# HaoxiangYou/Q_Learning_with_HJB

Measured on AMD Instinct MI355X. Metric: env-steps/sec (batched HJB rollouts), cartpole batch=2^20, higher is better.
Workload: dtype f32; 1 GPU; cartpole balancing + vhjb controller (BASELINE configs[1]); batch_per_gpu=1048576, global_batch=1048576, state_dim=4, control_dim=1, integrator=euler, mlp=4-128-128-64 relu, no bias, parallelism=env-shard x1, no data-path collective

## Files before the change

q_learning_with_hjb_amd/csrc/hjbx_mlp.hip:

```cpp
#include <hip/hip_runtime.h>
#include <type_traits>

#include <cstddef>

#include "hjbx_internal.hpp"
#include "hjbx_systems.hpp"
#include "hjbx_host.hpp"
#include "hjbx_mlp_core.hpp"
#include "hjbx_mlp_x3.hpp"
#include "hjbx_mlp_h2.hpp"
#include "hjbx_mlp_kernels.hpp"
#include "hjbx_mlp_host.hpp"

using namespace hjbx;

#ifndef HJBX_MLP_ACT
#error "compile hjbx_mlp.hip with -DHJBX_MLP_ACT=0 (relu + the C entry points), =1 (tanh), =2 (relu, bf16x3-split MFMA), =3 (relu, f16x2-split MFMA) and =4 (sin)"
#endif
static constexpr int kArith = HJBX_MLP_ACT == 2 ? 1 : HJBX_MLP_ACT == 3 ? 2 : 0;
static constexpr int kAct = kArith ? HJBX_ACT_RELU : HJBX_MLP_ACT == 4 ? HJBX_ACT_SIN : HJBX_MLP_ACT;
static_assert(kAct == HJBX_ACT_RELU || kAct == HJBX_ACT_TANH || kAct == HJBX_ACT_SIN, "fused kernels exist for relu, tanh and sin");
#define HJBX_MLP_CAT2(a, b) a##b
#define HJBX_MLP_CAT(a, b) HJBX_MLP_CAT2(a, b)
#define HJBX_MLP_SYM(name) HJBX_MLP_CAT(name, HJBX_MLP_ACT)
// ... 102 lines not shown
        return hjbx_user_value_grad(sys, &net, x, V, g, B, stream, "hjbx_value_grad_f32");
    }
    if (mlp->activation == HJBX_ACT_TANH) return hjbx_mlp_value_grad_act1(sys, mlp, x, V, g, B, stream);
    if (mlp->activation == HJBX_ACT_SIN) return hjbx_mlp_value_grad_act4(sys, mlp, x, V, g, B, stream);
    const int arith = hjbx_option_value(HJBX_OPT_MLP_ARITHMETIC);
    return arith == 1 ? hjbx_mlp_value_grad_act2(sys, mlp, x, V, g, B, stream)
         : arith == 2 ? hjbx_mlp_value_grad_act3(sys, mlp, x, V, g, B, stream)
                      : hjbx_mlp_value_grad_act0(sys, mlp, x, V, g, B, stream);
}
#endif

template <typename S>
static int launch_vhjb_rollout(const hjbx_system* sysh, S sys, const hjbx_task* task, const hjbx_mlp* mlp, int integrator, int t_first,
                               int n_steps, int T_max, const float* x, float* traj, float* u_log, float* cost, float* done, float* resid,
                               int32_t* done_step, float* x_out, const int32_t* order, int64_t B, void* workspace, void* st) {
    constexpr int N = S::N, M = S::M;
    constexpr int WAVES = HJBX_MLP_WAVES;
    const MlpP<N> p = make_mlp_params<N>(mlp->mean, mlp->std, mlp->xf, mlp->eps_scalar);
    const auto tk = make_task<float, N, M>(task);
    const auto lim = make_limits<float, M>(sysh);
    RolloutOut<N, M> o{traj, u_log, cost, done, resid, done_step, x_out};
    int64_t ngroups = 0, grid = 0;
    int sched = 0;
    if (int rc = mlp_rollout_grid(B, &ngroups, &grid, &sched, "hjbx_vhjb_rollout_f32")) return rc;
    const float *W1 = (const float*)mlp->W1, *W2 = (const float*)mlp->W2, *W3 = (const float*)mlp->W3;
    auto launch = [&](auto integ) {
        hipLaunchKernelGGL((k_vhjb_rollout_mfma<decltype(integ)::value, S, WAVES, kAct, kArith>), dim3((unsigned)grid), dim3(WAVES * 64), 0,
                           (hipStream_t)st, sys, p, tk, lim, W1, W2, W3, t_first, n_steps, T_max, x, order, o, B, ngroups, (unsigned*)workspace, sched, MlpHeadPd{});
    };
    if (integrator == HJBX_EULER) launch(std::integral_constant<int, 0>{});
    else if (integrator == HJBX_RK4) launch(std::integral_constant<int, 1>{});
    else if constexpr (S::kHasZoh) launch(std::integral_constant<int, 2>{});
    hipError_t e = hipGetLastError();
    if (e != hipSuccess) return hjbx_set_error(HJBX_EHIP, "hjbx_vhjb_rollout_f32: %s", hipGetErrorString(e));
    return HJBX_OK;
}

int HJBX_MLP_SYM(hjbx_mlp_rollout_act)(const hjbx_system* sys, const hjbx_task* task, const hjbx_mlp* mlp, int integrator, int t_first, int n_steps,
                                       int T_max, const float* x, float* traj, float* u_log, float* cost, float* done, float* resid,
                                       int32_t* done_step, float* x_out, const int32_t* env_order, int64_t B, void* workspace, void* stream) {
    int rc = HJBX_EUNSUPPORTED;
#ifdef HJBX_MLP_DEV
    if (sys->kind == HJBX_SYS_CARTPOLE && integrator == HJBX_EULER) {
        Cartpole<float> S{(float)sys->p[0], (float)sys->p[1], (float)sys->p[2], (float)sys->p[3]};
        constexpr int WAVES = HJBX_MLP_WAVES;
        MlpP<4> p;
        for (int k = 0; k < 4; ++k) { p.mean[k] = (float)mlp->mean[k]; p.istd[k] = (float)(1.0 / mlp->std[k]); p.xf[k] = (float)mlp->xf[k]; }
        p.eps_s = (float)mlp->eps_scalar;
        RolloutOut<4, 1> o{traj, u_log, cost, done, resid, done_step, x_out};
        const int64_t ngroups = (B + 31) / 32;
        int64_t grid = ngroups < 256 ? ngroups : 256;
        hipLaunchKernelGGL((k_vhjb_rollout_mfma<0, Cartpole<float>, WAVES, kAct, kArith>), dim3((unsigned)grid), dim3(WAVES * 64), 0, (hipStream_t)stream, S, p,
                           make_task<float, 4, 1>(task), make_limits<float, 1>(sys), (const float*)mlp->W1, (const float*)mlp->W2, (const float*)mlp->W3, t_first,
                           n_steps, T_max, x, env_order, o, B, ngroups, (unsigned*)workspace, hjbx_option_value(HJBX_OPT_ROLLOUT_SCHEDULE), MlpHeadPd{});
        return hipGetLastError() == hipSuccess ? HJBX_OK : hjbx_set_error(HJBX_EHIP, "launch");
    }
    return hjbx_set_error(HJBX_EUNSUPPORTED, "hjbx_vhjb_rollout_f32: development build (cartpole, Euler only)");
#else
    const bool ok = with_system<float>(sys, [&](auto S) {
        using SS = decltype(S);
        if constexpr (SS::N % 2 == 0)
            rc = launch_vhjb_rollout<SS>(sys, S, task, mlp, integrator, t_first, n_steps, T_max, x, traj, u_log, cost, done, resid, done_step,
                                         x_out, env_order, B, workspace, stream);
    });
    if (!ok || rc == HJBX_EUNSUPPORTED)
        return hjbx_set_error(HJBX_EUNSUPPORTED, "hjbx_vhjb_rollout_f32: no kernel for system kind %d with n=%d m=%d", sys->kind, sys->n, sys->m);
    return rc;
#endif
}

#if HJBX_MLP_ACT == 0
extern "C" int hjbx_vhjb_rollout_f32(const hjbx_system* sys, const hjbx_task* task, const hjbx_mlp* mlp, int integrator, int t_first,
                                     int n_steps, int T_max, const float* x, float* traj, float* u_log, float* cost, float* done,
// ... 40 lines not shown
```

q_learning_with_hjb_amd/csrc/hjbx_mlp_core.hpp:

```cpp
#pragma once
#include <hip/hip_runtime.h>

#include <cstddef>

#include "hjbx_internal.hpp"
#include "hjbx_systems.hpp"

using namespace hjbx;

using f32x16 = __attribute__((ext_vector_type(16))) float;
using f32x2 = __attribute__((ext_vector_type(2))) float;

static constexpr int kH1 = 128, kH2 = 128, kH3 = 64;
static constexpr int kLD1 = 129, kLD2 = 129, kLD3 = 65;

template <int N> struct MlpP { float mean[N], istd[N], xf[N], eps_s; };

__device__ __forceinline__ constexpr int perm(int s) { return (s & 3) + 8 * (s >> 2); }

#define MFMA(a, b, c) __builtin_amdgcn_mfma_f32_32x32x2f32((a), (b), (c), 0, 0, 0)

__device__ __forceinline__ float relu1(float v) {
    const int b = __builtin_bit_cast(int, v);
    return __builtin_bit_cast(float, b > 0 ? b : 0);
// ... 161 lines not shown
__device__ __forceinline__ void mlp_fill_bias(MlpBias& L, const float* __restrict__ b1g, const float* __restrict__ b2g, const float* __restrict__ b3g,
                                              const float* __restrict__ w4g, const float* __restrict__ b4g, int tid) {
    for (int idx = tid; idx < kH1; idx += THREADS) L.b1[idx] = b1g[idx];
    for (int idx = tid; idx < kH2; idx += THREADS) L.b2[idx] = b2g[idx];
    for (int idx = tid; idx < kH3; idx += THREADS) { L.b3[idx] = b3g[idx]; L.w4[idx] = w4g[idx]; }
    if (tid == 0) L.b4 = b4g[0];
}

template <int N> __device__ __forceinline__ MlpCtx mlp_ctx(MlpLds<N>& L, int lane) {
    constexpr int NP = MlpLds<N>::NP;
    MlpCtx c;
    c.i = lane & 31;
    c.h = lane >> 5;
    const uint32_t lds0 = (uint32_t)(uintptr_t)&L;
    c.w1f = lds0 + (uint32_t)offsetof(MlpLds<N>, W1) + 4u * (c.h * kLD1 + c.i);
    c.w2f = lds0 + (uint32_t)offsetof(MlpLds<N>, W2) + 4u * (4 * c.h * kLD2 + c.i);
    c.w3f = lds0 + (uint32_t)offsetof(MlpLds<N>, W3) + 4u * (4 * c.h * kLD3 + c.i);
    c.w3b = lds0 + (uint32_t)offsetof(MlpLds<N>, W3) + 4u * (c.i * kLD3 + 4 * c.h);
    c.w2b = lds0 + (uint32_t)offsetof(MlpLds<N>, W2) + 4u * (c.i * kLD2 + 4 * c.h);
    c.w1t = reinterpret_cast<const float4*>(L.W1T + 4 * c.h * NP);
    return c;
}

template <typename S, int TL, int ACT = HJBX_ACT_RELU, bool SOFT = false>
__device__ __forceinline__ void mlp_value_grad(const S& sys, const MlpP<S::N>& p, const MlpCtx& c, const float (&xs)[TL][S::N],
                                               bool want_grad, float (&V)[TL], float (&g)[TL][S::N], const MlpBias* bias = nullptr) {
    constexpr int N = S::N;
    constexpr int NP = MlpLds<N>::NP;
    const int h = c.h;
    float e[TL][N], z[TL][N], ee[TL];
#pragma unroll
    for (int t = 0; t < TL; ++t) {
        ee[t] = 0.f;
#pragma unroll
        for (int k = 0; k < N; ++k) e[t][k] = xs[t][k] - p.xf[k];
        sys.wrap(e[t]);
#pragma unroll
        for (int k = 0; k < N; ++k) {
            ee[t] += e[t][k] * e[t][k];
            z[t][k] = (e[t][k] - p.mean[k]) * p.istd[k];
        }
    }
    float ring4[3][4], ring2[3][2];

    f32x16 a1[TL][4];
    if constexpr (SOFT) bias_acc(a1, bias->b1, h);
    else zero_acc(a1);
    mfma_chain<OffW1F, N / 2, 4, 2, TL>(a1, ring4, c.w1f, [&](int st, int t) { return h ? z[t][2 * st + 1] : z[t][2 * st]; });


#pragma unroll
    for (int t = 0; t < TL; ++t)
#pragma unroll
        for (int fb = 0; fb < 4; ++fb)
#pragma unroll
            for (int r = 0; r < 16; ++r) {
                a1[t][fb][r] = act1<ACT>(a1[t][fb][r]);
                if constexpr (ACT == HJBX_ACT_SIN) {
                    asm volatile("" : "+v"(a1[t][fb][r]));
                    __builtin_amdgcn_sched_barrier(0);
                }
            }
    f32x16 a2[TL][4];
    if constexpr (SOFT) bias_acc(a2, bias->b2, h);
    else zero_acc(a2);
    mfma_chain<OffW2F, 64, 4, 2, TL>(a2, ring4, c.w2f, [&](int st, int t) { return a1[t][st >> 4][st & 15]; });

    f32x16 c2[ACT == HJBX_ACT_SIN ? TL : 1][ACT == HJBX_ACT_SIN ? 4 : 1];
#pragma unroll
    for (int t = 0; t < TL; ++t)
#pragma unroll
// ... 27 lines not shown
                for (int q = 0; q < 4; ++q) {
                    const float4 w = *reinterpret_cast<const float4*>(bias->w4 + 32 * ob + 8 * q + 4 * h);
                    const float wv[4] = {w.x, w.y, w.z, w.w};
                    float hv[4];
#pragma unroll
                    for (int j = 0; j < 4; ++j) {
                        const float a = y[t][ob][4 * q + j];
                        if constexpr (ACT == HJBX_ACT_SIN) {
                            float sn, cs;
                            sincos1(a, sn, cs);
                            asm volatile("" : "+v"(sn), "+v"(cs));
                            hv[j] = sn;
                            y[t][ob][4 * q + j] = cs * wv[j];
                            __builtin_amdgcn_sched_barrier(0);
                        } else {
                            hv[j] = act1<ACT>(a);
                            y[t][ob][4 * q + j] = dact1<ACT>(hv[j], wv[j]);
                        }
                    }
                    acc2 = __builtin_elementwise_fma(f32x2{hv[0], hv[1]}, f32x2{wv[0], wv[1]}, acc2);
                    acc2 = __builtin_elementwise_fma(f32x2{hv[2], hv[3]}, f32x2{wv[2], wv[3]}, acc2);
                }
            vpart[t] = acc2[0] + acc2[1];
            V[t] = vpart[t] + __shfl_xor(vpart[t], 32, 64) + bias->b4;
        }
    } else {
#pragma unroll
    for (int t = 0; t < TL; ++t) {
        f32x2 acc2{0.f, 0.f};
#pragma unroll
        for (int ob = 0; ob < 2; ++ob)
#pragma unroll
            for (int r = 0; r < 16; r += 2) {
                const f32x2 yy{y[t][ob][r], y[t][ob][r + 1]};
                acc2 = __builtin_elementwise_fma(yy, yy, acc2);
                const f32x2 y2 = yy + yy;
                y[t][ob][r] = y2[0];
                y[t][ob][r + 1] = y2[1];
            }
        vpart[t] = acc2[0] + acc2[1];
        V[t] = vpart[t] + __shfl_xor(vpart[t], 32, 64) + p.eps_s * ee[t];
    }
    }
    if (!want_grad) return;

    f32x16 d2[TL][4];
    zero_acc(d2);
    mfma_chain<OffW3B, 32, 4, 2, TL>(d2, ring4, c.w3b, [&](int st, int t) { return y[t][st >> 4][st & 15]; });

#pragma unroll
    for (int t = 0; t < TL; ++t)
#pragma unroll
        for (int fb = 0; fb < 4; ++fb)
#pragma unroll
            for (int r = 0; r < 16; ++r) d2[t][fb][r] = dact1<ACT>(ACT == HJBX_ACT_SIN ? c2[ACT == HJBX_ACT_SIN ? t : 0][ACT == HJBX_ACT_SIN ? fb : 0][r] : a2[t][fb][r], d2[t][fb][r]);
    f32x16 d1[TL][4];
    zero_acc(d1);
    mfma_chain<OffW2B, 64, 4, 2, TL>(d1, ring4, c.w2b, [&](int st, int t) { return d2[t][st >> 4][st & 15]; });

    if constexpr (SOFT) bias_acc(a1, bias->b1, h);
    else zero_acc(a1);
    mfma_chain<OffW1F, N / 2, 4, 2, TL>(a1, ring4, c.w1f, [&](int st, int t) { return h ? z[t][2 * st + 1] : z[t][2 * st]; });
#pragma unroll
    for (int t = 0; t < TL; ++t) {
        f32x2 part[NP / 2];
#pragma unroll
        for (int k = 0; k < NP / 2; ++k) part[k] = f32x2{0.f, 0.f};
#pragma unroll
        for (int kb = 0; kb < 4; ++kb)
#pragma unroll
            for (int s = 0; s < 16; ++s) {
                float dv = dact1<ACT>(ACT == HJBX_ACT_RELU ? a1[t][kb][s] : ACT == HJBX_ACT_SIN ? cos1(a1[t][kb][s]) : act1<ACT>(a1[t][kb][s]), d1[t][kb][s]);
                if constexpr (ACT == HJBX_ACT_SIN) {
                    asm volatile("" : "+v"(dv));
                    __builtin_amdgcn_sched_barrier(0);
                }
                const f32x2 dv2{dv, dv};
#pragma unroll
                for (int q = 0; q < NP / 4; ++q) {
                    const float4 w = c.w1t[(32 * kb + perm(s)) * (NP / 4) + q];
                    part[2 * q + 0] = __builtin_elementwise_fma(f32x2{w.x, w.y}, dv2, part[2 * q + 0]);
                    part[2 * q + 1] = __builtin_elementwise_fma(f32x2{w.z, w.w}, dv2, part[2 * q + 1]);
                }
            }
#pragma unroll
        for (int k = 0; k < N; ++k) {
            const float pk = part[k >> 1][k & 1];
            const float v = pk + __shfl_xor(pk, 32, 64);
            if constexpr (SOFT) g[t][k] = v * p.istd[k];
            else g[t][k] = v * p.istd[k] + 2.f * p.eps_s * e[t][k];
        }
    }
}

template <int N> __device__ __forceinline__ void load_row(const float* __restrict__ x, int64_t env, float (&dst)[N]) {
    if constexpr ((N * 4) % 16 == 0) {
        const float4* rp = reinterpret_cast<const float4*>(x + env * N);
#pragma unroll
        for (int q = 0; q < N / 4; ++q) {
            const float4 v = rp[q];
            dst[4 * q] = v.x; dst[4 * q + 1] = v.y; dst[4 * q + 2] = v.z; dst[4 * q + 3] = v.w;
        }
    } else {
        const float2* rp2 = reinterpret_cast<const float2*>(x + env * N);
#pragma unroll
        for (int q = 0; q < N / 2; ++q) {
            const float2 v = rp2[q];
            dst[2 * q] = v.x; dst[2 * q + 1] = v.y;
        }
    }
}

template <int N> __device__ __forceinline__ void store_row(float* __restrict__ out, int64_t env, const float (&src)[N]) {
    if constexpr ((N * 4) % 16 == 0) {
        float4* op = reinterpret_cast<float4*>(out + env * N);
// ... 13 lines not shown
```

q_learning_with_hjb_amd/csrc/hjbx_mlp_host.hpp:

```cpp
#pragma once
#include "hjbx_host.hpp"
#include "hjbx_mlp_kernels.hpp"

template <int N> inline MlpP<N> make_mlp_params(const double* mean, const double* std, const double* xf, double eps_scalar) {
    MlpP<N> p;
    for (int k = 0; k < N; ++k) { p.mean[k] = (float)mean[k]; p.istd[k] = (float)(1.0 / std[k]); p.xf[k] = (float)xf[k]; }
    p.eps_s = (float)eps_scalar;
    return p;
}

inline int mlp_value_grad_grid(int64_t B, int TL, int64_t* ngroups, int64_t* grid, const char* who) {
    *ngroups = (B + 32 * TL - 1) / (32 * TL);
    const int n_cu = hjbx_device_cus();
    if (n_cu <= 0) return hjbx_set_error(HJBX_ENODEVICE, "%s: no HIP device", who);
    *grid = *ngroups < n_cu ? *ngroups : n_cu;
    return HJBX_OK;
}

inline int mlp_rollout_grid(int64_t B, int64_t* ngroups, int64_t* grid, int* sched, const char* who) {
    if (int rc = mlp_value_grad_grid(B, 1, ngroups, grid, who)) return rc;
    *sched = hjbx_option_value(HJBX_OPT_ROLLOUT_SCHEDULE);
    *grid += hjbx_option_value(HJBX_OPT_ROLLOUT_EXTRA_WORKGROUPS);
    if (*grid > kMaxGrid) *grid = kMaxGrid;
    return HJBX_OK;
}
```

q_learning_with_hjb_amd/csrc/hjbx_mlp_kernels.hpp:

```cpp
#pragma once
#include <hip/hip_runtime.h>
#include <type_traits>

#include <cstddef>

#include "hjbx_internal.hpp"
#include "hjbx_systems.hpp"
#include "hjbx_mlp_core.hpp"
#include "hjbx_mlp_x3.hpp"
#include "hjbx_mlp_h2.hpp"

using namespace hjbx;

template <int N, int AR> using MlpLdsT = std::conditional_t<AR == 1, MlpLdsX3<N>, std::conditional_t<AR == 2, MlpLdsH2<N>, MlpLds<N>>>;

struct MlpHeadPd {
    static constexpr bool kSoft = false;
    template <int N, int AR> using Lds = MlpLdsT<N, AR>;
};
struct MlpHeadSoft {
    static constexpr bool kSoft = true;
    template <int N, int AR> using Lds = MlpLdsSoft<N>;
    const float *b1, *b2, *b3, *w4, *b4;
};
// ... 84 lines not shown
        }
    }
#endif
}

template <int N, int M> struct RolloutOut {
    float* traj;
    float* u_log;
    float* cost;
    float* done;
    float* resid;
    int32_t* done_step;
    float* x_out;
};

static constexpr int kWsQueue = 0;
static constexpr int kWsStarted = 32;
static constexpr int kWsExited = 64;
static constexpr int kWsFlags = 96;
static constexpr int kMaxGrid = 1024;
static constexpr int kWsOpen = kWsFlags + kMaxGrid;
static constexpr int kWsWords = kWsOpen + kMaxGrid;
#define HJBX_RLX_AGENT __ATOMIC_RELAXED, __HIP_MEMORY_SCOPE_AGENT

template <int INTEG, typename S, int WAVES, int ACT, int AR, typename HEAD = MlpHeadPd>
__global__ __launch_bounds__(WAVES * 64, WAVES / 4) void k_vhjb_rollout_mfma(S sys_k, MlpP<S::N> p_k, TaskP<float, S::N, S::M> tk_k,
                                                                           Limits<float, S::M> lim_k, const float* __restrict__ W1g,
                                                                           const float* __restrict__ W2g, const float* __restrict__ W3g,
                                                                           int t_first, int n_steps, int T_max, const float* x ,
                                                                           const int32_t* __restrict__ order, RolloutOut<S::N, S::M> o, int64_t B,
                                                                           int64_t ngroups, unsigned* ws, int sched, HEAD head) {
    constexpr int N = S::N, M = S::M;
    static_assert(N % 2 == 0, "state dimension must be even (k-steps of 2)");
    __shared__ __attribute__((aligned(256))) typename HEAD::template Lds<N, AR> L;
    __shared__ __attribute__((aligned(16))) unsigned char sys_raw[sizeof(S)];
    S& sys_s = *reinterpret_cast<S*>(sys_raw);
    __shared__ MlpP<N> p_s;
    __shared__ TaskP<float, N, M> tk_s;
    __shared__ Limits<float, M> lim_s;
    const int tid = threadIdx.x;
    __shared__ int q_next[4];
    __shared__ int waves_done;
    __shared__ unsigned my_flag;
    if (tid < 4) q_next[tid] = WAVES / 4;
    if (tid == 0) {
        waves_done = 0;
// ... 50 lines not shown
            const int w = victim + lane;
            unsigned f = 1u;
            if (w < G) {
                f = __hip_atomic_load(ws + kWsFlags + w, HJBX_RLX_AGENT);
                if (f == 0u && __hip_atomic_compare_exchange_strong(ws + kWsFlags + w, &f, 2u, __ATOMIC_RELAXED, HJBX_RLX_AGENT)) f = 2u;
            }
            unsigned long long open = __builtin_amdgcn_ballot_w64(f == 2u);
            while (open) {
                const int b = __builtin_ctzll(open);
                unsigned t = 0;
                if (lane == 0) t = __hip_atomic_fetch_add(ws + kWsOpen + victim + b, 1u, HJBX_RLX_AGENT);
                const int64_t g = group_of(victim + b, (int64_t)(unsigned)__builtin_amdgcn_readfirstlane((int)t));
                if (g >= 0) { victim += b; return g; }
                open &= open - 1;
            }
            victim = (victim + 64 < G) ? victim + 64 : G;
        }
        return -1;
    };
    int64_t grp;
    if (sched == 1) grp = (int64_t)blockIdx.x * WAVES + wave < ngroups ? (int64_t)blockIdx.x * WAVES + wave : -1;
    else grp = my_flag_u == 0u ? group_of(blockIdx.x, wave) : -1;
    if (grp < 0) grp = next_group();
    while (grp >= 0) {
        const int64_t slot = grp * 32 + i;
        const bool valid = slot < B;
        int64_t env = valid ? (order ? (int64_t)order[slot] : slot) : 0;
        env = env < 0 ? 0 : (env >= B ? B - 1 : env);
        const bool writer = valid && h == 0;
        float xs[1][N];
        int32_t ds = 0;
        if (valid) {
            load_row<N>(x, env, xs[0]);
            ds = o.done_step[env];
        } else {
#pragma unroll
            for (int k = 0; k < N; ++k) xs[0][k] = p.xf[k];
        }
        if (o.traj && writer) store_row<N>(o.traj, env, xs[0]);
        for (int k = 0; k < n_steps; ++k) {
            asm volatile("" ::: "memory");
            float xo[N], u[M], cst, dn, res;
            if (__builtin_amdgcn_ballot_w64(ds < 0) == 0) {
#pragma unroll
                for (int q = 0; q < N; ++q) xo[q] = xs[0][q];
#pragma unroll
                for (int j = 0; j < M; ++j) u[j] = 0.0f;
                cst = dn = res = 0.0f;
            } else {
                float V[1], g[1][N];
                if constexpr (AR == 1) mlp_value_grad_x3<S>(sys, p, c, xs, true, V, g);
                else if constexpr (AR == 2) mlp_value_grad_h2<S>(sys, p, c, xs, true, V, g);
                else if constexpr (HEAD::kSoft) mlp_value_grad<S, 1, ACT, true>(sys, p, c, xs, true, V, g, &L.bias);
                else mlp_value_grad<S, 1, ACT>(sys, p, c, xs, true, V, g);
                vhjb_step_env<INTEG>(sys, tk, lim, t_first + k, T_max, o.resid != nullptr, xs[0], g[0], ds, xo, u, cst, dn, res);
            }
            if (writer) {
                const int64_t row = (int64_t)k * B + env;
                o.cost[row] = cst;
                o.done[row] = dn;
                if (o.resid) o.resid[row] = res;
                if (o.u_log) store_row<M>(o.u_log + (int64_t)k * B * M, env, u);
                if (o.traj) store_row<N>(o.traj + (int64_t)(k + 1) * B * N, env, xo);
            }
#pragma unroll
            for (int q = 0; q < N; ++q) xs[0][q] = xo[q];
// ... 15 lines not shown
```

q_learning_with_hjb_amd/csrc/hjbx_softpd.hip:

```cpp
#include <hip/hip_runtime.h>
#include <type_traits>

#include "hjbx_internal.hpp"
#include "hjbx_systems.hpp"
#include "hjbx_host.hpp"
#include "hjbx_mlp_kernels.hpp"
#include "hjbx_mlp_host.hpp"

using namespace hjbx;

#ifndef HJBX_SOFTPD_ACT
#error "compile hjbx_softpd.hip with -DHJBX_SOFTPD_ACT=0 (relu + the C entry points), =1 (tanh) and =2 (sin)"
#endif
static constexpr int kAct = HJBX_SOFTPD_ACT;
static_assert(kAct == HJBX_ACT_RELU || kAct == HJBX_ACT_TANH || kAct == HJBX_ACT_SIN, "soft-PD kernels exist for relu, tanh and sin");
#define HJBX_SOFTPD_CAT2(a, b) a##b
#define HJBX_SOFTPD_CAT(a, b) HJBX_SOFTPD_CAT2(a, b)
#define HJBX_SOFTPD_SYM(name) HJBX_SOFTPD_CAT(name, HJBX_SOFTPD_ACT)
#define HJBX_HIDDEN __attribute__((visibility("hidden")))
static constexpr int kWaves = 8;

#define HJBX_SOFTPD_VG_ARGS const hjbx_system*, const hjbx_softpd_mlp*, const float*, float*, float*, int64_t, void*
#define HJBX_SOFTPD_RO_ARGS                                                                                                                 \
    const hjbx_system*, const hjbx_task*, const hjbx_softpd_mlp*, int, int, int, int, const float*, float*, float*, float*, float*, float*, \
// ... 33 lines not shown
        if (sys->n == 2) { Linear<float, 2, 1> l{}; return launch_softpd_value_grad(l, mlp, x, V, g, B, stream); }
        if (sys->n == 4) { Linear<float, 4, 1> l{}; return launch_softpd_value_grad(l, mlp, x, V, g, B, stream); }
        if (sys->n == 6) { Linear<float, 6, 2> l{}; return launch_softpd_value_grad(l, mlp, x, V, g, B, stream); }
        break;
    case HJBX_SYS_CARTPOLE: { Cartpole<float> c{}; return launch_softpd_value_grad(c, mlp, x, V, g, B, stream); }
    case HJBX_SYS_ACROBOT: { Acrobot<float> a{}; return launch_softpd_value_grad(a, mlp, x, V, g, B, stream); }
    case HJBX_SYS_QUAD2D: { Quad2D<float> q{}; return launch_softpd_value_grad(q, mlp, x, V, g, B, stream); }
    case HJBX_SYS_NEARHOVER: { NearHover<float> q{}; return launch_softpd_value_grad(q, mlp, x, V, g, B, stream); }
    }
    return hjbx_set_error(HJBX_EUNSUPPORTED, "hjbx_softpd_value_grad_f32: no kernel for system kind %d with n=%d", sys->kind, sys->n);
}

template <typename S>
static int launch_softpd_rollout(const hjbx_system* sysh, S sys, const hjbx_task* task, const hjbx_softpd_mlp* mlp, int integrator, int t_first,
                                 int n_steps, int T_max, const float* x, float* traj, float* u_log, float* cost, float* done, float* resid,
                                 int32_t* done_step, float* x_out, const int32_t* order, int64_t B, void* workspace, void* st) {
    constexpr int N = S::N, M = S::M;
    const MlpP<N> p = softpd_params<N>(mlp);
    const auto tk = make_task<float, N, M>(task);
    const auto lim = make_limits<float, M>(sysh);
    RolloutOut<N, M> o{traj, u_log, cost, done, resid, done_step, x_out};
    int64_t ngroups = 0, grid = 0;
    int sched = 0;
    if (int rc = mlp_rollout_grid(B, &ngroups, &grid, &sched, "hjbx_softpd_rollout_f32")) return rc;
    const float *W1 = (const float*)mlp->W1, *W2 = (const float*)mlp->W2, *W3 = (const float*)mlp->W3;
    auto launch = [&](auto integ) {
        hipLaunchKernelGGL((k_vhjb_rollout_mfma<decltype(integ)::value, S, kWaves, kAct, 0, MlpHeadSoft>), dim3((unsigned)grid), dim3(kWaves * 64), 0,
                           (hipStream_t)st, sys, p, tk, lim, W1, W2, W3, t_first, n_steps, T_max, x, order, o, B, ngroups, (unsigned*)workspace, sched,
                           softpd_head(mlp));
    };
    if (integrator == HJBX_EULER) launch(std::integral_constant<int, 0>{});
    else if (integrator == HJBX_RK4) launch(std::integral_constant<int, 1>{});
    else if constexpr (S::kHasZoh) launch(std::integral_constant<int, 2>{});
    hipError_t e = hipGetLastError();
    if (e != hipSuccess) return hjbx_set_error(HJBX_EHIP, "hjbx_softpd_rollout_f32: %s", hipGetErrorString(e));
    return HJBX_OK;
}

int HJBX_SOFTPD_SYM(hjbx_softpd_rollout_act)(const hjbx_system* sys, const hjbx_task* task, const hjbx_softpd_mlp* mlp, int integrator, int t_first,
                                             int n_steps, int T_max, const float* x, float* traj, float* u_log, float* cost, float* done, float* resid,
                                             int32_t* done_step, float* x_out, const int32_t* env_order, int64_t B, void* workspace, void* stream) {
    int rc = HJBX_EUNSUPPORTED;
    const bool ok = with_system<float>(sys, [&](auto S) {
        using SS = decltype(S);
        if constexpr (SS::N % 2 == 0)
            rc = launch_softpd_rollout<SS>(sys, S, task, mlp, integrator, t_first, n_steps, T_max, x, traj, u_log, cost, done, resid, done_step, x_out,
                                           env_order, B, workspace, stream);
// ... 77 lines not shown
```

q_learning_with_hjb_amd/csrc/hjbx_systems.hpp:

```cpp
#pragma once
#include <hip/hip_runtime.h>
#include <stdint.h>

namespace hjbx {

#define HJBX_DEV __device__ __forceinline__

template <typename T> struct Const;
template <> struct Const<float> {
    static constexpr float pi = 3.14159274101257324219f;
    static constexpr float two_pi = 6.28318548202514648438f;
};
template <> struct Const<double> {
    static constexpr double pi = 3.14159265358979311600;
    static constexpr double two_pi = 6.28318530717958623200;
};

HJBX_DEV void sincos_t(float a, float* s, float* c) { sincosf(a, s, c); }
HJBX_DEV void sincos_t(double a, double* s, double* c) { sincos(a, s, c); }
HJBX_DEV float tan_t(float a) { return tanf(a); }
HJBX_DEV double tan_t(double a) { return tan(a); }
HJBX_DEV float fmod_t(float a, float b) { return fmodf(a, b); }
HJBX_DEV double fmod_t(double a, double b) { return fmod(a, b); }
HJBX_DEV float sqrt_t(float a) { return sqrtf(a); }
// ... 4 lines not shown
template <typename T> HJBX_DEV T wrap_angle(T th) {
    constexpr T pi = Const<T>::pi, b = Const<T>::two_pi;
    const T a = th + pi;
    T r;
    if (a >= T(0) && a < b) r = a;
    else if (a >= b && a < T(2) * b) r = a - b;
    else if (a < T(0) && a >= -b) r = a + b;
    else {
        r = fmod_t(a, b);
        if (r != T(0)) { if (r < T(0)) r += b; } else r = T(0);
    }
    return r - pi;
}

template <typename T> HJBX_DEV T clamp_t(T v, T lo, T hi) {
    v = v < lo ? lo : v;
    v = v > hi ? hi : v;
    return v;
}

template <typename T, int N_, int M_> struct Linear {
    static constexpr int N = N_, M = M_;
    static constexpr bool kHasZoh = true;
    T A[N * N], Bm[N * M];
    T Ad[N * N], Bd[N * M];
    HJBX_DEV void wrap(T*) const {}
    HJBX_DEV void zoh_step(const T* x, const T* u, T* xn) const {
#pragma unroll
        for (int i = 0; i < N; ++i) {
            T acc = T(0);
#pragma unroll
            for (int j = 0; j < N; ++j) acc += Ad[i * N + j] * x[j];
            T bu = T(0);
#pragma unroll
            for (int j = 0; j < M; ++j) bu += Bd[i * M + j] * u[j];
            xn[i] = acc + bu;
        }
    }
    HJBX_DEV void affine(const T* x, T* f1, T* f2) const {
#pragma unroll
        for (int i = 0; i < N; ++i) {
            T acc = T(0);
#pragma unroll
            for (int j = 0; j < N; ++j) acc += A[i * N + j] * x[j];
            f1[i] = acc;
#pragma unroll
            for (int j = 0; j < M; ++j) f2[i * M + j] = Bm[i * M + j];
        }
    }
    HJBX_DEV void xdot(const T* x, const T* u, T* xd) const {
#pragma unroll
        for (int i = 0; i < N; ++i) {
            T acc = T(0);
#pragma unroll
            for (int j = 0; j < N; ++j) acc += A[i * N + j] * x[j];
            T bu = T(0);
#pragma unroll
            for (int j = 0; j < M; ++j) bu += Bm[i * M + j] * u[j];
            xd[i] = acc + bu;
        }
    }
};

template <typename T> struct Cartpole {
    static constexpr bool kHasZoh = false;
    static constexpr int N = 4, M = 1;
    T mc, mp, l, g;
    T il = T(1) / l;
    HJBX_DEV T over_l(T v) const {
        if constexpr (sizeof(T) == 4) return v * il;
        else return v / l;
    }
    HJBX_DEV void wrap(T* x) const { x[1] = wrap_angle(x[1]); }
    HJBX_DEV void affine(const T* x, T* f1, T* f2) const {
        T s, c;
        sincos_t(x[1], &s, &c);
        const T invD = T(1) / (mc + mp * s * s);
        const T w = mp * l * x[3] * x[3] * s;
        f1[0] = x[2];
        f1[1] = x[3];
        f1[2] = (w + mp * g * s * c) * invD;
        f1[3] = over_l(-(w * c + (mc + mp) * g * s) * invD);
        f2[0] = T(0);
        f2[1] = T(0);
        f2[2] = invD;
        f2[3] = over_l(-c * invD);
    }
    HJBX_DEV void xdot(const T* x, const T* u, T* xd) const {
        T f1[4], f2[4];
        affine(x, f1, f2);
#pragma unroll
        for (int i = 0; i < 4; ++i) xd[i] = f1[i] + f2[i] * u[0];
    }
};

template <typename T> struct Acrobot {
    static constexpr bool kHasZoh = false;
    static constexpr int N = 4, M = 1;
    T m1, m2, l1, l2, I1, I2, g;
    HJBX_DEV void wrap(T* x) const { x[0] = wrap_angle(x[0]); x[1] = wrap_angle(x[1]); }
    HJBX_DEV void mch(const T* x, T& a, T& b, T& d, T& h0, T& h1) const {
        T s1, c1, s2, c2, s12, c12;
        sincos_t(x[0], &s1, &c1);
        sincos_t(x[1], &s2, &c2);
        sincos_t(x[0] + x[1], &s12, &c12);
        const T k = m2 * l1 * l2 / T(2);
        a = I1 + I2 + m2 * l1 * l1 + T(2) * k * c2;
        b = I2 + k * c2;
        d = I2;
        const T G0 = (m1 * l1 / T(2) + m2 * l1) * g * s1 + m2 * g * l2 / T(2) * s12;
        const T G1 = m2 * g * l2 / T(2) * s12;
        h0 = (-T(2) * k * s2 * x[3]) * x[2] + (-k * s2 * x[3]) * x[3] + G0;
        h1 = (k * s2 * x[2]) * x[2] + G1;
    }
    HJBX_DEV T energy(const T* x) const {
        T s1, c1, s2, c2, s12, c12;
        sincos_t(x[0], &s1, &c1);
        sincos_t(x[1], &s2, &c2);
        sincos_t(x[0] + x[1], &s12, &c12);
        const T k = m2 * l1 * l2 / T(2);
// ... 6 lines not shown
    HJBX_DEV void affine(const T* x, T* f1, T* f2) const {
        T a, b, d, h0, h1;
        mch(x, a, b, d, h0, h1);
        const T idet = T(1) / (a * d - b * b);
        f1[0] = x[2];
        f1[1] = x[3];
        f1[2] = -(d * h0 - b * h1) * idet;
        f1[3] = -(-b * h0 + a * h1) * idet;
        f2[0] = T(0);
        f2[1] = T(0);
        f2[2] = -b * idet;
        f2[3] = a * idet;
    }
    HJBX_DEV void xdot(const T* x, const T* u, T* xd) const {
        T f1[4], f2[4];
        affine(x, f1, f2);
#pragma unroll
        for (int i = 0; i < 4; ++i) xd[i] = f1[i] + f2[i] * u[0];
    }
};

template <typename T> struct Quad2D {
    static constexpr bool kHasZoh = false;
    static constexpr int N = 6, M = 2;
    T m, r, I, g;
    T im = T(1) / m, rI = r / I;
    HJBX_DEV T over_m(T v) const {
        if constexpr (sizeof(T) == 4) return v * im;
        else return v / m;
    }
    HJBX_DEV T r_over_I() const {
        if constexpr (sizeof(T) == 4) return rI;
        else return r / I;
    }
    HJBX_DEV void wrap(T* x) const { x[2] = wrap_angle(x[2]); }
    HJBX_DEV void affine(const T* x, T* f1, T* f2) const {
        T s, c;
        sincos_t(x[2], &s, &c);
        f1[0] = x[3]; f1[1] = x[4]; f1[2] = x[5]; f1[3] = T(0); f1[4] = -g; f1[5] = T(0);
#pragma unroll
        for (int i = 0; i < 6; ++i) f2[i] = T(0);
        f2[6] = over_m(-s); f2[7] = over_m(-s);
        f2[8] = over_m(c);  f2[9] = over_m(c);
        f2[10] = r_over_I(); f2[11] = -r_over_I();
    }
    HJBX_DEV void xdot(const T* x, const T* u, T* xd) const {
        T s, c;
        sincos_t(x[2], &s, &c);
        xd[0] = x[3]; xd[1] = x[4]; xd[2] = x[5];
        xd[3] = T(0) + (over_m(-s) * u[0] + over_m(-s) * u[1]);
        xd[4] = -g + (over_m(c) * u[0] + over_m(c) * u[1]);
        xd[5] = T(0) + (r_over_I() * u[0] + (-r_over_I()) * u[1]);
    }
};

template <typename T> struct NearHover {
    static constexpr bool kHasZoh = false;
    static constexpr int N = 10, M = 3;
    T g, m, kT, n0;
    T kTm_f = kT / m;
    HJBX_DEV T kT_over_m() const {
        if constexpr (sizeof(T) == 4) return kTm_f;
        else return kT / m;
    }
    HJBX_DEV void wrap(T* x) const { x[3] = wrap_angle(x[3]); x[4] = wrap_angle(x[4]); }
    HJBX_DEV void affine(const T* x, T* f1, T* f2) const {
#pragma unroll
        for (int i = 0; i < 5; ++i) f1[i] = x[5 + i];
        f1[5] = g * tan_t(x[3]); f1[6] = g * tan_t(x[4]); f1[7] = -g; f1[8] = T(0); f1[9] = T(0);
#pragma unroll
        for (int i = 0; i < 30; ++i) f2[i] = T(0);
        f2[21] = kT_over_m(); f2[25] = n0; f2[29] = n0;
    }
    HJBX_DEV void xdot(const T* x, const T* u, T* xd) const {
#pragma unroll
        for (int i = 0; i < 5; ++i) xd[i] = x[5 + i];
        xd[5] = g * tan_t(x[3]);
        xd[6] = g * tan_t(x[4]);
        xd[7] = -g + kT_over_m() * u[0];
        xd[8] = n0 * u[1];
// ... 291 lines not shown
```

q_learning_with_hjb_amd/csrc/hjbx_user.hip:

```cpp
#include <hip/hip_runtime.h>
#include <hip/hiprtc.h>

#include <dlfcn.h>
#include <elf.h>

#include <cstdio>
#include <cstring>
#include <map>
#include <mutex>
#include <new>
#include <string>
#include <vector>

#include "hjbx_internal.hpp"
#include "hjbx_host.hpp"
#include "hjbx_mlp_kernels.hpp"
#include "hjbx_mlp_host.hpp"

#if !defined(__HIP_DEVICE_COMPILE__)
#ifndef HJBX_CSRC_DIR
#error "compile hjbx_user.hip with -DHJBX_CSRC_DIR=\"<absolute path of csrc>\""
#endif
#define HJBX_EMBED(sym, file)                                                                                                     \
    asm(".pushsection .rodata\n.global " #sym "\n.type " #sym ", @object\n" #sym ":\n.incbin \"" HJBX_CSRC_DIR "/" file "\"\n.byte 0\n" \
// ... 428 lines not shown
        MlpHeadSoft soft = user_head(net);
        MlpHeadPd pd{};
        void* a[] = {&blob, &p, (void*)&net->W1, (void*)&net->W2, (void*)&net->W3, (void*)&x, (void*)&V, (void*)&g, (void*)&B, &ngroups,
                     net->soft ? (void*)&soft : (void*)&pd};
        return launch_unit(static_cast<UserProgram*>(s->user), *unit, unit->kernel[0].c_str(), (unsigned)grid, kMcBlock, a, stream, who);
    });
}

int hjbx_user_rollout(const hjbx_system* s, const hjbx_task* task, const hjbx_user_net* net, int integrator, int t_first, int n_steps, int T_max,
                      const float* x, float* traj, float* u_log, float* cost, float* done, float* resid, int32_t* done_step, float* x_out,
                      const int32_t* order, int64_t B, void* workspace, void* stream, const char* who) {
    if (integrator != HJBX_EULER && integrator != HJBX_RK4) return hjbx_set_error(HJBX_EUNSUPPORTED, "%s: a user system steps with HJBX_EULER or HJBX_RK4", who);
    UserUnit* unit = nullptr;
    if (int rc = matrix_core_unit(s, net->soft, net->activation, who, &unit)) return rc;
    return with_mc_dims(s, who, [&](auto Nc, auto Mc) -> int {
        constexpr int N = decltype(Nc)::value, M = decltype(Mc)::value;
        UserBlobF blob = user_blob(s);
        MlpP<N> p = make_mlp_params<N>(net->mean, net->std, net->xf, net->eps_scalar);
        auto tk = make_task<float, N, M>(task);
        auto lim = make_limits<float, M>(s);
        RolloutOut<N, M> o{traj, u_log, cost, done, resid, done_step, x_out};
        int64_t ngroups = 0, grid = 0;
        int sched = 0;
        if (int rc = mlp_rollout_grid(B, &ngroups, &grid, &sched, who)) return rc;
        unsigned* ws = (unsigned*)workspace;
        MlpHeadSoft soft = user_head(net);
        MlpHeadPd pd{};
        void* a[] = {&blob, &p, &tk, &lim, (void*)&net->W1, (void*)&net->W2, (void*)&net->W3, &t_first, &n_steps, &T_max, (void*)&x, (void*)&order,
                     &o, (void*)&B, &ngroups, &ws, &sched, net->soft ? (void*)&soft : (void*)&pd};
        return launch_unit(static_cast<UserProgram*>(s->user), *unit, unit->kernel[integrator == HJBX_RK4 ? 2 : 1].c_str(), (unsigned)grid, kMcBlock, a,
                           stream, who);
    });
}

int hjbx_user_train_unit(const hjbx_system* s, int activation, const char* who) {
    UserUnit* unit = nullptr;
    return train_unit(s, activation, who, &unit);
}

int hjbx_user_train_launch(const hjbx_system* s, int activation, int mode, int psplit, unsigned grid, void** args, void* stream, const char* who) {
    if (mode < 0 || mode > 1 || (psplit != 1 && psplit != 4)) return hjbx_set_error(HJBX_EINVAL, "%s: residual mode %d / psplit %d", who, mode, psplit);
    UserUnit* unit = nullptr;
    if (int rc = train_unit(s, activation, who, &unit)) return rc;
    UserBlobF blob = user_blob(s);
    args[0] = &blob;
    return launch_unit(static_cast<UserProgram*>(s->user), *unit, unit->kernel[2 * mode + (psplit == 4 ? 1 : 0)].c_str(), grid, 256, args, stream, who);
}
// ... 1 lines not shown
```

Before: 1.424 billion env-steps/s.

## Give each wave lane its own env and run the MLP in two half-wave passes

Before this change, each wave handled 32 environments, with both half-waves holding the same env and the per-env dynamics and error work repeated. Now each of the 64 lanes owns one env (64 envs per wave). For each half, the normalized state is redistributed with permlane32_swap and the MFMA value/grad core runs in two passes. A pass is skipped when all 32 envs in that half are done. To support this, mlp_value_grad is split into reusable pieces (error/z, core, grad_x), and the grid sizing takes a group size. The aim is to remove the duplicated scalar dynamics and bookkeeping per env. In exchange it adds a serialized two-pass loop, lane-swap traffic and more register pressure.

```diff
diff --git a/q_learning_with_hjb_amd/csrc/hjbx_mlp.hip b/q_learning_with_hjb_amd/csrc/hjbx_mlp.hip
--- a/q_learning_with_hjb_amd/csrc/hjbx_mlp.hip
+++ b/q_learning_with_hjb_amd/csrc/hjbx_mlp.hip
@@ -148,7 +148,7 @@
     RolloutOut<N, M> o{traj, u_log, cost, done, resid, done_step, x_out};
     int64_t ngroups = 0, grid = 0;
     int sched = 0;
-    if (int rc = mlp_rollout_grid(B, &ngroups, &grid, &sched, "hjbx_vhjb_rollout_f32")) return rc;
+    if (int rc = mlp_rollout_grid(B, kRolloutGroup<S, kArith>, &ngroups, &grid, &sched, "hjbx_vhjb_rollout_f32")) return rc;
     const float *W1 = (const float*)mlp->W1, *W2 = (const float*)mlp->W2, *W3 = (const float*)mlp->W3;
     auto launch = [&](auto integ) {
         hipLaunchKernelGGL((k_vhjb_rollout_mfma<decltype(integ)::value, S, WAVES, kAct, kArith>), dim3((unsigned)grid), dim3(WAVES * 64), 0,
@@ -174,7 +174,8 @@
         for (int k = 0; k < 4; ++k) { p.mean[k] = (float)mlp->mean[k]; p.istd[k] = (float)(1.0 / mlp->std[k]); p.xf[k] = (float)mlp->xf[k]; }
         p.eps_s = (float)mlp->eps_scalar;
         RolloutOut<4, 1> o{traj, u_log, cost, done, resid, done_step, x_out};
-        const int64_t ngroups = (B + 31) / 32;
+        constexpr int GROUP = kRolloutGroup<Cartpole<float>, kArith>;
+        const int64_t ngroups = (B + GROUP - 1) / GROUP;
         int64_t grid = ngroups < 256 ? ngroups : 256;
         hipLaunchKernelGGL((k_vhjb_rollout_mfma<0, Cartpole<float>, WAVES, kAct, kArith>), dim3((unsigned)grid), dim3(WAVES * 64), 0, (hipStream_t)stream, S, p,
                            make_task<float, 4, 1>(task), make_limits<float, 1>(sys), (const float*)mlp->W1, (const float*)mlp->W2, (const float*)mlp->W3, t_first,
diff --git a/q_learning_with_hjb_amd/csrc/hjbx_mlp_core.hpp b/q_learning_with_hjb_amd/csrc/hjbx_mlp_core.hpp
--- a/q_learning_with_hjb_amd/csrc/hjbx_mlp_core.hpp
+++ b/q_learning_with_hjb_amd/csrc/hjbx_mlp_core.hpp
@@ -207,31 +207,25 @@
     return c;
 }
 
-template <typename S, int TL, int ACT = HJBX_ACT_RELU, bool SOFT = false>
-__device__ __forceinline__ void mlp_value_grad(const S& sys, const MlpP<S::N>& p, const MlpCtx& c, const float (&xs)[TL][S::N],
-                                               bool want_grad, float (&V)[TL], float (&g)[TL][S::N], const MlpBias* bias = nullptr) {
-    constexpr int N = S::N;
+template <typename S> __device__ __forceinline__ void mlp_error_z(const S& sys, const MlpP<S::N>& p, const float (&x)[S::N], float (&e)[S::N], float (&z)[S::N]) {
+#pragma unroll
+    for (int k = 0; k < S::N; ++k) e[k] = x[k] - p.xf[k];
+    sys.wrap(e);
+#pragma unroll
+    for (int k = 0; k < S::N; ++k) z[k] = (e[k] - p.mean[k]) * p.istd[k];
+}
+
+template <int N, int TL, int ACT, bool SOFT, typename GetZ>
+__device__ __forceinline__ void mlp_value_grad_core(const MlpCtx& c, GetZ getZ, bool want_grad, float (&vsum)[TL], float (&gz)[TL][N],
+                                                    const MlpBias* bias) {
     constexpr int NP = MlpLds<N>::NP;
     const int h = c.h;
-    float e[TL][N], z[TL][N], ee[TL];
-#pragma unroll
-    for (int t = 0; t < TL; ++t) {
-        ee[t] = 0.f;
-#pragma unroll
-        for (int k = 0; k < N; ++k) e[t][k] = xs[t][k] - p.xf[k];
-        sys.wrap(e[t]);
-#pragma unroll
-        for (int k = 0; k < N; ++k) {
-            ee[t] += e[t][k] * e[t][k];
-            z[t][k] = (e[t][k] - p.mean[k]) * p.istd[k];
-        }
-    }
     float ring4[3][4], ring2[3][2];
 
     f32x16 a1[TL][4];
     if constexpr (SOFT) bias_acc(a1, bias->b1, h);
     else zero_acc(a1);
-    mfma_chain<OffW1F, N / 2, 4, 2, TL>(a1, ring4, c.w1f, [&](int st, int t) { return h ? z[t][2 * st + 1] : z[t][2 * st]; });
+    mfma_chain<OffW1F, N / 2, 4, 2, TL>(a1, ring4, c.w1f, getZ);
 
 
 #pragma unroll
@@ -305,7 +299,7 @@
                     acc2 = __builtin_elementwise_fma(f32x2{hv[2], hv[3]}, f32x2{wv[2], wv[3]}, acc2);
                 }
             vpart[t] = acc2[0] + acc2[1];
-            V[t] = vpart[t] + __shfl_xor(vpart[t], 32, 64) + bias->b4;
+            vsum[t] = vpart[t] + __shfl_xor(vpart[t], 32, 64);
         }
     } else {
 #pragma unroll
@@ -322,7 +316,7 @@
                 y[t][ob][r + 1] = y2[1];
             }
         vpart[t] = acc2[0] + acc2[1];
-        V[t] = vpart[t] + __shfl_xor(vpart[t], 32, 64) + p.eps_s * ee[t];
+        vsum[t] = vpart[t] + __shfl_xor(vpart[t], 32, 64);
     }
     }
     if (!want_grad) return;
@@ -343,7 +337,7 @@
 
     if constexpr (SOFT) bias_acc(a1, bias->b1, h);
     else zero_acc(a1);
-    mfma_chain<OffW1F, N / 2, 4, 2, TL>(a1, ring4, c.w1f, [&](int st, int t) { return h ? z[t][2 * st + 1] : z[t][2 * st]; });
+    mfma_chain<OffW1F, N / 2, 4, 2, TL>(a1, ring4, c.w1f, getZ);
 #pragma unroll
     for (int t = 0; t < TL; ++t) {
         f32x2 part[NP / 2];
@@ -369,11 +363,42 @@
 #pragma unroll
         for (int k = 0; k < N; ++k) {
             const float pk = part[k >> 1][k & 1];
-            const float v = pk + __shfl_xor(pk, 32, 64);
-            if constexpr (SOFT) g[t][k] = v * p.istd[k];
-            else g[t][k] = v * p.istd[k] + 2.f * p.eps_s * e[t][k];
-        }
-    }
+            gz[t][k] = pk + __shfl_xor(pk, 32, 64);
+        }
+    }
+}
+
+template <int N, bool SOFT> __device__ __forceinline__ void mlp_grad_x(const MlpP<N>& p, const float (&gz)[N], const float (&e)[N], float (&g)[N]) {
+#pragma unroll
+    for (int k = 0; k < N; ++k) {
+        const float v = gz[k];
+        if constexpr (SOFT) g[k] = v * p.istd[k];
+        else g[k] = v * p.istd[k] + 2.f * p.eps_s * e[k];
+    }
+}
+
+template <typename S, int TL, int ACT = HJBX_ACT_RELU, bool SOFT = false>
+__device__ __forceinline__ void mlp_value_grad(const S& sys, const MlpP<S::N>& p, const MlpCtx& c, const float (&xs)[TL][S::N],
+                                               bool want_grad, float (&V)[TL], float (&g)[TL][S::N], const MlpBias* bias = nullptr) {
+    constexpr int N = S::N;
+    const int h = c.h;
+    float e[TL][N], z[TL][N], ee[TL], vsum[TL], gz[TL][N];
+#pragma unroll
+    for (int t = 0; t < TL; ++t) {
+        mlp_error_z<S>(sys, p, xs[t], e[t], z[t]);
+        ee[t] = 0.f;
+#pragma unroll
+        for (int k = 0; k < N; ++k) ee[t] += e[t][k] * e[t][k];
+    }
+    mlp_value_grad_core<N, TL, ACT, SOFT>(c, [&](int st, int t) { return h ? z[t][2 * st + 1] : z[t][2 * st]; }, want_grad, vsum, gz, bias);
+#pragma unroll
+    for (int t = 0; t < TL; ++t) {
+        if constexpr (SOFT) V[t] = vsum[t] + bias->b4;
+        else V[t] = vsum[t] + p.eps_s * ee[t];
+    }
+    if (!want_grad) return;
+#pragma unroll
+    for (int t = 0; t < TL; ++t) mlp_grad_x<N, SOFT>(p, gz[t], e[t], g[t]);
 }
 
 template <int N> __device__ __forceinline__ void load_row(const float* __restrict__ x, int64_t env, float (&dst)[N]) {
diff --git a/q_learning_with_hjb_amd/csrc/hjbx_mlp_host.hpp b/q_learning_with_hjb_amd/csrc/hjbx_mlp_host.hpp
--- a/q_learning_with_hjb_amd/csrc/hjbx_mlp_host.hpp
+++ b/q_learning_with_hjb_amd/csrc/hjbx_mlp_host.hpp
@@ -17,8 +17,8 @@
     return HJBX_OK;
 }
 
-inline int mlp_rollout_grid(int64_t B, int64_t* ngroups, int64_t* grid, int* sched, const char* who) {
-    if (int rc = mlp_value_grad_grid(B, 1, ngroups, grid, who)) return rc;
+inline int mlp_rollout_grid(int64_t B, int group, int64_t* ngroups, int64_t* grid, int* sched, const char* who) {
+    if (int rc = mlp_value_grad_grid(B, group / 32, ngroups, grid, who)) return rc;
     *sched = hjbx_option_value(HJBX_OPT_ROLLOUT_SCHEDULE);
     *grid += hjbx_option_value(HJBX_OPT_ROLLOUT_EXTRA_WORKGROUPS);
     if (*grid > kMaxGrid) *grid = kMaxGrid;
diff --git a/q_learning_with_hjb_amd/csrc/hjbx_mlp_kernels.hpp b/q_learning_with_hjb_amd/csrc/hjbx_mlp_kernels.hpp
--- a/q_learning_with_hjb_amd/csrc/hjbx_mlp_kernels.hpp
+++ b/q_learning_with_hjb_amd/csrc/hjbx_mlp_kernels.hpp
@@ -130,6 +130,11 @@
 static constexpr int kWsOpen = kWsFlags + kMaxGrid;
 static constexpr int kWsWords = kWsOpen + kMaxGrid;
 #define HJBX_RLX_AGENT __ATOMIC_RELAXED, __HIP_MEMORY_SCOPE_AGENT
+
+template <typename S> constexpr auto rollout_pairs_of(int) -> decltype(S::kRolloutPairs) { return S::kRolloutPairs; }
+template <typename S> constexpr bool rollout_pairs_of(...) { return false; }
+template <typename S, int AR> static constexpr bool kRolloutPairs = AR == 0 && rollout_pairs_of<S>(0);
+template <typename S, int AR> static constexpr int kRolloutGroup = kRolloutPairs<S, AR> ? 64 : 32;
 
 template <int INTEG, typename S, int WAVES, int ACT, int AR, typename HEAD = MlpHeadPd>
 __global__ __launch_bounds__(WAVES * 64, WAVES / 4) void k_vhjb_rollout_mfma(S sys_k, MlpP<S::N> p_k, TaskP<float, S::N, S::M> tk_k,
@@ -226,12 +231,13 @@
     if (sched == 1) grp = (int64_t)blockIdx.x * WAVES + wave < ngroups ? (int64_t)blockIdx.x * WAVES + wave : -1;
     else grp = my_flag_u == 0u ? group_of(blockIdx.x, wave) : -1;
     if (grp < 0) grp = next_group();
+    constexpr bool PAIR = kRolloutPairs<S, AR>;
     while (grp >= 0) {
-        const int64_t slot = grp * 32 + i;
+        const int64_t slot = PAIR ? grp * 64 + lane : grp * 32 + i;
         const bool valid = slot < B;
         int64_t env = valid ? (order ? (int64_t)order[slot] : slot) : 0;
         env = env < 0 ? 0 : (env >= B ? B - 1 : env);
-        const bool writer = valid && h == 0;
+        const bool writer = valid && (PAIR || h == 0);
         float xs[1][N];
         int32_t ds = 0;
         if (valid) {
@@ -245,7 +251,43 @@
         for (int k = 0; k < n_steps; ++k) {
             asm volatile("" ::: "memory");
             float xo[N], u[M], cst, dn, res;
-            if (__builtin_amdgcn_ballot_w64(ds < 0) == 0) {
+            if constexpr (PAIR) {
+                const unsigned long long live = __builtin_amdgcn_ballot_w64(ds < 0);
+                if (live == 0) {
+#pragma unroll
+                    for (int q = 0; q < N; ++q) xo[q] = xs[0][q];
+#pragma unroll
+                    for (int j = 0; j < M; ++j) u[j] = 0.0f;
+                    cst = dn = res = 0.0f;
+                } else {
+                    float e[N], z[N], zab[2][N / 2], gz[N], g[N];
+                    mlp_error_z<S>(sys, p, xs[0], e, z);
+#pragma unroll
+                    for (int st = 0; st < N / 2; ++st) {
+                        const auto r = __builtin_amdgcn_permlane32_swap(__builtin_bit_cast(unsigned, z[2 * st]), __builtin_bit_cast(unsigned, z[2 * st + 1]), false, false);
+                        zab[0][st] = __builtin_bit_cast(float, r[0]);
+                        zab[1][st] = __builtin_bit_cast(float, r[1]);
+                    }
+#pragma unroll
+                    for (int q = 0; q < N; ++q) gz[q] = 0.f;
+#pragma nounroll
+                    for (int pass = 0; pass < 2; ++pass) {
+                        asm volatile("" ::: "memory");
+                        if ((unsigned)(live >> (32 * pass)) == 0u) continue;
+                        float zb[N / 2], vsum[1], gp[1][N];
+#pragma unroll
+                        for (int st = 0; st < N / 2; ++st) zb[st] = pass ? zab[1][st] : zab[0][st];
+                        mlp_value_grad_core<N, 1, ACT, HEAD::kSoft>(c, [&](int st, int) { return zb[st]; }, true, vsum, gp, [&]() -> const MlpBias* {
+                            if constexpr (HEAD::kSoft) return &L.bias;
+                            else return nullptr;
+                        }());
+#pragma unroll
+                        for (int q = 0; q < N; ++q) gz[q] = h == pass ? gp[0][q] : gz[q];
+                    }
+                    mlp_grad_x<N, HEAD::kSoft>(p, gz, e, g);
+                    vhjb_step_env<INTEG>(sys, tk, lim, t_first + k, T_max, o.resid != nullptr, xs[0], g, ds, xo, u, cst, dn, res);
+                }
+            } else if (__builtin_amdgcn_ballot_w64(ds < 0) == 0) {
 #pragma unroll
                 for (int q = 0; q < N; ++q) xo[q] = xs[0][q];
 #pragma unroll
diff --git a/q_learning_with_hjb_amd/csrc/hjbx_softpd.hip b/q_learning_with_hjb_amd/csrc/hjbx_softpd.hip
--- a/q_learning_with_hjb_amd/csrc/hjbx_softpd.hip
+++ b/q_learning_with_hjb_amd/csrc/hjbx_softpd.hip
@@ -79,7 +79,7 @@
     RolloutOut<N, M> o{traj, u_log, cost, done, resid, done_step, x_out};
     int64_t ngroups = 0, grid = 0;
     int sched = 0;
-    if (int rc = mlp_rollout_grid(B, &ngroups, &grid, &sched, "hjbx_softpd_rollout_f32")) return rc;
+    if (int rc = mlp_rollout_grid(B, kRolloutGroup<S, 0>, &ngroups, &grid, &sched, "hjbx_softpd_rollout_f32")) return rc;
     const float *W1 = (const float*)mlp->W1, *W2 = (const float*)mlp->W2, *W3 = (const float*)mlp->W3;
     auto launch = [&](auto integ) {
         hipLaunchKernelGGL((k_vhjb_rollout_mfma<decltype(integ)::value, S, kWaves, kAct, 0, MlpHeadSoft>), dim3((unsigned)grid), dim3(kWaves * 64), 0,
diff --git a/q_learning_with_hjb_amd/csrc/hjbx_systems.hpp b/q_learning_with_hjb_amd/csrc/hjbx_systems.hpp
--- a/q_learning_with_hjb_amd/csrc/hjbx_systems.hpp
+++ b/q_learning_with_hjb_amd/csrc/hjbx_systems.hpp
@@ -50,6 +50,7 @@
 template <typename T, int N_, int M_> struct Linear {
     static constexpr int N = N_, M = M_;
     static constexpr bool kHasZoh = true;
+    static constexpr bool kRolloutPairs = true;
     T A[N * N], Bm[N * M];
     T Ad[N * N], Bd[N * M];
     HJBX_DEV void wrap(T*) const {}
@@ -92,6 +93,7 @@
 
 template <typename T> struct Cartpole {
     static constexpr bool kHasZoh = false;
+    static constexpr bool kRolloutPairs = true;
     static constexpr int N = 4, M = 1;
     T mc, mp, l, g;
     T il = T(1) / l;
@@ -124,6 +126,7 @@
 
 template <typename T> struct Acrobot {
     static constexpr bool kHasZoh = false;
+    static constexpr bool kRolloutPairs = true;
     static constexpr int N = 4, M = 1;
     T m1, m2, l1, l2, I1, I2, g;
     HJBX_DEV void wrap(T* x) const { x[0] = wrap_angle(x[0]); x[1] = wrap_angle(x[1]); }
@@ -176,6 +179,7 @@
 
 template <typename T> struct Quad2D {
     static constexpr bool kHasZoh = false;
+    static constexpr bool kRolloutPairs = true;
     static constexpr int N = 6, M = 2;
     T m, r, I, g;
     T im = T(1) / m, rI = r / I;
@@ -210,6 +214,7 @@
 
 template <typename T> struct NearHover {
     static constexpr bool kHasZoh = false;
+    static constexpr bool kRolloutPairs = true;
     static constexpr int N = 10, M = 3;
     T g, m, kT, n0;
     T kTm_f = kT / m;
diff --git a/q_learning_with_hjb_amd/csrc/hjbx_user.hip b/q_learning_with_hjb_amd/csrc/hjbx_user.hip
--- a/q_learning_with_hjb_amd/csrc/hjbx_user.hip
+++ b/q_learning_with_hjb_amd/csrc/hjbx_user.hip
@@ -474,7 +474,7 @@
         RolloutOut<N, M> o{traj, u_log, cost, done, resid, done_step, x_out};
         int64_t ngroups = 0, grid = 0;
         int sched = 0;
-        if (int rc = mlp_rollout_grid(B, &ngroups, &grid, &sched, who)) return rc;
+        if (int rc = mlp_rollout_grid(B, 32, &ngroups, &grid, &sched, who)) return rc;
         unsigned* ws = (unsigned*)workspace;
         MlpHeadSoft soft = user_head(net);
         MlpHeadPd pd{};
```

Result: slower. 609.1 million env-steps/s (-57.2%).
